# killerwhile/kafka-assignment-optimizer

Measured on AMD Instinct MI355X. Metric: candidate assignments/sec (+ time_to_optimal_s), 10k-partition reassign, higher is better.
Workload: dtype int32

## Files before the change

### kafka_assignment_optimizer_amd/csrc/kao_search.hip

```cpp
#include "kao_search_dev.h"

namespace kao {

template <bool kGlobalA, bool kPriced, int NW, bool kWide, bool kTeam, bool kCurG = false, int RFT = 0, bool kSmall = false>
__device__ __forceinline__ void search_body(unsigned char *smem, const SearchPools &pl, const SearchParams &prm) {
    static_assert(!kTeam || kGlobalA, "teams run topics that live in global memory");
    static_assert(!kCurG || !kGlobalA, "kCurG: the working assignment is in LDS");
    static_assert(RFT == 0 || (RFT == 3 && NW == 4 && !kGlobalA && !kTeam), "RFT = 3: LDS-resident topics of four words per partition");
    static_assert(!kSmall || (RFT == 3 && !kPriced && !kCurG), "kSmall: the unpriced RF-3 instantiation");
    constexpr int NS = RFT ? RFT : NW;
    const int lane = threadIdx.x & 63;
    const int wave = __builtin_amdgcn_readfirstlane(threadIdx.x >> 6);
    const int n_waves = kTeam ? __builtin_amdgcn_readfirstlane((int)(blockDim.x >> 6)) : 1;
    const int tid = kTeam ? (int)threadIdx.x : lane, nthr = kTeam ? (int)blockDim.x : 64;
    const int2 bm = pl.block_map[blockIdx.x];
    const TopicDev *TD = pl.topics + bm.x;

    TopicRegs T = topic_regs<RFT>(TD);
    {
        uint32_t v0 = T.c7_inc, v1 = T.c7_dec;
        asm volatile("" : "+v"(v0), "+v"(v1));
        T.c7_inc = (uint32_t)__builtin_amdgcn_readfirstlane((int)v0); T.c7_dec = (uint32_t)__builtin_amdgcn_readfirstlane((int)v1);
    }
    constexpr bool kBandTabs = kSmall;
// ... 157 lines not shown
    const int plog = TD->period_log2 + (rho & 3);
    const uint32_t pmask = (1u << plog) - 1u;
    const uint32_t lrange = (uint32_t)(prm.lam_max - prm.lam_min + 1);
    const uint32_t RF8 = (uint32_t)T.RF << 8, R8 = (uint32_t)T.R << 8, m8 = (uint32_t)T.m << 8;

    const int T_tour = min(64, max(4, (T.P * T.RF) >> 2));
    uint32_t tour_off = lane < T_tour ? 0u : kKeyNull;
    asm volatile("" : "+v"(tour_off));
    const int GA = min(16, max(1, (T.P * T.RF) >> 8));
    const int x_rounds_full = (T.P + 63) >> 6;
    const bool x_windowed = x_rounds_full > 8;

    int lam_lo = prm.lam_min, lam_hi = prm.lam_max;
    uint32_t n_iters = prm.iters, it_base = prm.launch * prm.iters;
    constexpr uint32_t kLpScanTwo = 1u << 29;
    uint32_t loop_pack = TD->P * TD->RF <= prm.scan2_max ? kLpScanTwo : 0u;
    if (kSmall) loop_pack |= ((uint32_t)prm.lam_min & 0xFFFu) | (((uint32_t)prm.lam_max & 0xFFFu) << 12) | (((uint32_t)plog & 31u) << 24);
    {
        uint32_t v0 = (uint32_t)lam_lo, v1 = (uint32_t)lam_hi, v2 = n_iters, v3 = it_base, v4 = loop_pack;
        asm volatile("" : "+v"(v2), "+v"(v3), "+v"(v4));
        if constexpr (!kSmall) {
            asm volatile("" : "+v"(v0), "+v"(v1));
            lam_lo = (int)__builtin_amdgcn_readfirstlane(v0); lam_hi = (int)__builtin_amdgcn_readfirstlane(v1);
        }
        n_iters = __builtin_amdgcn_readfirstlane(v2); it_base = __builtin_amdgcn_readfirstlane(v3);
        loop_pack = __builtin_amdgcn_readfirstlane(v4);
    }
    auto loop_flag = [&](uint32_t bit) { uint32_t lp = loop_pack; asm volatile("" : "+s"(lp)); return (lp & bit) != 0u; };
    constexpr bool kFuse = !kGlobalA && !kTeam && !kPriced;
    const bool fuse_ok = kFuse && T.Bx <= 16384;
    uint32_t jmp_a = 1u, jmp_c = 0u;
    if (fuse_ok)
        for (int n = (T.Bx + 63) >> 6; n > 0; --n) { jmp_a = (jmp_a * 0x6D2B79u) & 0xFFFFFFu; jmp_c = (jmp_c * 0x6D2B79u + 0x3C6EF3u) & 0xFFFFFFu; }
    best_obj = __builtin_amdgcn_readfirstlane(best_obj);
    for (uint32_t i = 0; i < n_iters; ++i) {
        const uint32_t it = it_base + i;
        const int type = (int)((0x1210u >> ((it & 7u) * 2u)) & 3u);
        int lam;
        if constexpr (kSmall) {
            uint32_t lp = loop_pack;
            asm volatile("" : "+s"(lp));
            const uint32_t plg = (lp >> 24) & 31u;
            const int lo_ = (int)(lp & 0xFFFu), hi_ = (int)((lp >> 12) & 0xFFFu);
            const uint32_t ph = it & ((1u << plg) - 1u);
            lam = best_obj < 0 ? hi_ : min(hi_, lo_ + (int)((2u * ph * (uint32_t)(hi_ - lo_ + 1)) >> plg));
        } else {
            const uint32_t ph = it & pmask;
            lam = best_obj < 0 ? lam_hi : min(lam_hi, lam_lo + (int)((2u * ph * lrange) >> plog));
        }
        const bool sampled = (type == 2) || (type == 0 && ((it >> 3) & 1u));

        auto finish = [&](auto ty, auto uni, uint32_t kmin, int win, int p, int k, int q, int j, uint32_t uw, uint32_t vw, int dV, int dObj) {
            constexpr int TY = decltype(ty)::value;
            auto of_win = [&](int v) { return decltype(uni)::value ? v : __builtin_amdgcn_readlane(v, win); };
            if (!kTeam) {
                if (kmin == kKeyNull) return;
                if ((int)(kmin >> 8) - kDBias > 0) return;
            }
            bool mine = true;
            int *rec = TR + ((i & 1u) * 16 + (uint32_t)wave) * kTeamRec;
            if (kTeam) {
                const bool ok = kmin != kKeyNull && (int)(kmin >> 8) - kDBias <= 0;
                if (lane == win) {
                    const uint32_t ro_ = uw >> 16, rn_ = vw >> 16;
                    const bool racks = ok && TY == 0 && ro_ != rn_;
                    rec[0] = ok ? 1 : 0; rec[1] = p; rec[2] = TY == 1 ? q : p;
                    rec[3] = (int)(uw & 0xFFFFu); rec[4] = (int)(vw & 0xFFFFu);
                    rec[5] = racks ? (int)ro_ : 0xFFFF; rec[6] = racks ? (int)rn_ : 0xFFFF;
                    rec[7] = dV; rec[8] = dObj;
                }
                __syncthreads();
                bool clash = false;
                if (lane < wave) {
                    const int *o = TR + ((i & 1u) * 16 + (uint32_t)lane) * kTeamRec;
                    if (o[0]) {
                        const int mp = rec[1], mq = rec[2], mb0 = rec[3], mb1 = rec[4], mr0 = rec[5], mr1 = rec[6];
                        clash = (o[1] == mp) | (o[1] == mq) | (o[2] == mp) | (o[2] == mq) | (o[3] == mb0) | (o[3] == mb1) | (o[4] == mb0) | (o[4] == mb1);
                        if (o[5] != 0xFFFF && mr0 != 0xFFFF) clash |= (o[5] == mr0) | (o[5] == mr1) | (o[6] == mr0) | (o[6] == mr1);
                    }
                }
                mine = ok && __ballot(clash) == 0ull;
            }

            if (lane == win && mine) {
                uint32_t *ap = reinterpret_cast<uint32_t *>(&L.A[p]);
                if (TY == 0) {
                    const uint32_t d = (k == 0) ? 0x10001u : 1u;
                    L.C[uw & 0xFFFFu] -= d;
                    L.C[vw & 0xFFFFu] += d;
                    if (!kTeam || (uw >> 16) != (vw >> 16)) {
                        L.K[uw >> 16] -= 1;
                        L.K[vw >> 16] += 1;
                    }
                    ap[k] = vw;
                } else if (TY == 1) {
                    uint32_t *bp = reinterpret_cast<uint32_t *>(&L.A[q]);
                    if ((k == 0) != (j == 0)) {
                        const uint32_t lose = (k == 0) ? uw : vw, gain = (k == 0) ? vw : uw;
                        L.C[lose & 0xFFFFu] -= 0x10000u;
                        L.C[gain & 0xFFFFu] += 0x10000u;
                    }
                    ap[k] = vw;
                    bp[j] = uw;
                } else {
                    L.C[uw & 0xFFFFu] -= 0x10000u;
                    L.C[vw & 0xFFFFu] += 0x10000u;
                    ap[0] = vw;
                    ap[k] = uw;
                }
            }
            if (mine) {
                int rows;
                if (TY == 0) rows = 1 | (of_win(k) == 0 ? 2 : 0);
                else if (TY == 1) rows = (of_win(k) == 0 ? 2 : 0) ^ (of_win(j) == 0 ? 2 : 0);
                else rows = 2;
                if (rows != 0) {
                    const uint32_t xo = (uint32_t)of_win((int)uw) & 0xFFFFu, xn = decltype(uni)::value ? (uint32_t)__builtin_amdgcn_readfirstlane((int)(vw & 0xFFFFu)) : (uint32_t)of_win((int)vw) & 0xFFFFu;
                    uint32_t xx = xo;
                    asm("v_writelane_b32 %0, %1, 1" : "+v"(xx) : "s"(xn));
                    int lane_w = lane;
                    asm volatile("" : "+v"(lane_w));
                    if (lane_w < 2) {
                        const uint32_t cx = L.C[xx];
                        uint32_t wx;
                        if (rows == 3) wx = band_row<kBandTabs>((int)(cx & 0xFFFFu), bq_r0, bq_r1) | (band_row<kBandTabs>((int)(cx >> 16), bq_l0, bq_l1) << 6);
                        else if (rows == 1) wx = (L.W[xx] & ~kWRowR) | band_row<kBandTabs>((int)(cx & 0xFFFFu), bq_r0, bq_r1);
                        else wx = (L.W[xx] & ~kWRowL) | (band_row<kBandTabs>((int)(cx >> 16), bq_l0, bq_l1) << 6);
                        L.W[xx] = (uint16_t)wx;
                    }
                }
            }
            if (kGlobalA) __builtin_amdgcn_fence(__ATOMIC_SEQ_CST, "workgroup");
            if (kTeam) {
                if (lane == 0) rec[9] = mine ? 1 : 0;
                __syncthreads();
                int dVs = 0, dOs = 0, na = 0;
                if (lane < n_waves) {
                    const int *o = TR + ((i & 1u) * 16 + (uint32_t)lane) * kTeamRec;
                    if (o[9]) { dVs = o[7]; dOs = o[8]; na = 1; }
                }
                V += wave_sum(dVs);
                obj += wave_sum(dOs);
                accepted += wave_sum(na);
            } else {
                V += of_win(dV);
                obj += of_win(dObj);
                accepted++;
            }
        };
        constexpr std::integral_constant<int, 0> kReplace{};
        constexpr std::integral_constant<int, 1> kExchange{};
        constexpr std::integral_constant<int, 2> kLeaderSwap{};

        if (sampled) {
            const int p = (int)rnd24_wide(rng, (uint32_t)T.P);
            const Part<NW> a = L.A[p];
            const Part<NW> c = CUR[p];
            uint32_t key = kKeyNull, vw = 0;
            int dV = 0, dObj = 0;
            if (type == 0) {
                const int k = (int)rnd24(rng, RF8);
                const uint32_t uw = sel_slot<NS>(a, k);
                const uint32_t ro = uw >> 16;
                const bool lead = k == 0;
                const uint32_t lw = lead ? 2u : 0u;
                const int wl = lead ? T.w00 : T.w01, wf = lead ? T.w10 : T.w11;
                const int g_old = role_w2<NS>(c, uw, wl, wf) + (hbw ? bw_of(BW[uw & 0xFFFFu], lead) : 0);
                const uint32_t wo = L.W[uw & 0xFFFFu];
                const int dV_old = wfld(wo, kWDecR) + wfldw(wo, kWDecL, lw);
                const int dV_rack_old = ddec(L.K[ro], T.rack_lo, T.rack_hi) + c7_delta(T.c7_dec, cnt4x2<NS>(a, ro));
                const int rsz_ro = RSZ[ro];
                int dP_old = 0, dP_rack_old = 0;
                if (kPriced) {
                    const uint32_t pro = PR[uw & 0xFFFFu];
                    dP_old = -(wflag(wo, kWPoutR) & price_rep(pro));
                    if (lead) dP_old -= wflag(wo, kWPoutL) & price_lead(pro);
                    dP_rack_old = p_out(L.K[ro], T.rack_lo, T.rack_hi, PG[ro]);
                }
                const int base_s = kSmall ? mad24s(S, g_old, kDBias) : 0;
#pragma unroll
                for (int g = 0; g < 4; ++g) {
                    uint32_t r, jj;
                    bool okg;
                    if (g < 2) {
                        r = rnd24(rng, R8);
                        jj = rnd24(rng, m8);
                        okg = (int)jj < RSZ[r];
                    } else {
                        r = ro;
                        jj = rnd24(rng, (uint32_t)rsz_ro << 8);
                        okg = true;
                    }
                    const uint32_t x = __umul24(r, (uint32_t)T.m) + jj;
                    const uint32_t xw = x | (r << 16);
                    okg = okg && !in4<NS>(a, xw);
                    const uint32_t wn = L.W[x];
                    int dVg = dV_old + wfld(wn, kWIncR) + wfldw(wn, kWIncL, lw);
                    if (g < 2) {
                        if (r != ro)
                            dVg += dV_rack_old + dinc(L.K[r], T.rack_lo, T.rack_hi) + c7_delta(T.c7_inc, cnt4x2<NS>(a, r));
                    }
                    const int dObjg = role_w2<NS>(c, xw, wl, wf) + (hbw ? bw_of(BW[x], lead) : 0) - (kSmall ? 0 : g_old);
                    uint32_t keyg;
                    if constexpr (kSmall) keyg = okg ? key_small(mad24s(-S, dObjg, mad24s(lam, dVg, base_s)), (uint32_t)lane) : kKeyNull;
                    else if (kPriced) {
                        const uint32_t prx = PR[x];
                        int dPg = dP_old + (wflag(wn, kWPinR) & price_rep(prx));
                        if (lead) dPg += wflag(wn, kWPinL) & price_lead(prx);
                        if (g < 2 && r != ro) dPg += dP_rack_old + p_in(L.K[r], T.rack_lo, T.rack_hi, PG[r]);
                        keyg = okg ? make_key_p(lam, S, dVg, dObjg, dPg, lane) : kKeyNull;
                    }
                    else keyg = okg ? make_key(lam, S, dVg, dObjg, lane) : kKeyNull;
                    if (keyg < key) { key = keyg; vw = xw; dV = dVg; dObj = dObjg; }
// ... 108 lines not shown
                    const int q_draw = (int)rnd24_wide(rng, (uint32_t)T.P);
                    q0 = x_windowed ? __builtin_amdgcn_readfirstlane(q_draw) : 0;
#pragma unroll
                    for (int r2 = 0; r2 < XB; ++r2) { int qq; bool okq; const int qc = x_partner(r2, qq, okq); xb[r2] = L.A[qc]; xcb[r2] = CUR[qc]; }
                }
#pragma unroll
                for (int g0 = 0; g0 < 16; g0 += TB) {
                    if (g0 > 0 && g0 >= GA) break;
                    Part<NW> tal[TB], tcl[TB];
                    int tp[TB];
#pragma unroll
                    for (int g = 0; g < TB; ++g) { tp[g] = (g0 + g) < GA ? part(g0 + g) : p0; tal[g] = L.A[tp[g]]; tcl[g] = CUR[tp[g]]; }
#pragma unroll
                    for (int g = 0; g < TB; ++g) {
                        uint32_t kg, ow;
                        int gg, d1 = 0, d2 = 0;
                        score_words(ty, kg, tal[g], tcl[g], kk[g0 + g], ow, gg, d1, d2);
                        if (g0 + g > 0) kg |= (g0 + g) < GA ? 0u : kKeyNull;
                        if (g0 + g == 0 || kg < keyA) { keyA = kg; pl_ = tp[g]; kl_ = kk[g0 + g]; oldw_l = ow; g_old_l = gg; dvo_l = d1; dvr_l = d2; a_l = tal[g]; c_l = tcl[g]; }
                    }
                }
            };
            if constexpr (kGlobalA) { if (type == 0) tournament_global(std::integral_constant<int, 0>{}); else tournament_global(std::integral_constant<int, 1>{}); }
            else if (type == 0) tournament(std::integral_constant<int, 0>{}); else tournament(std::integral_constant<int, 1>{});
            const int wA1 = (int)(wave_umin(keyA) & 63u);
            int wA2 = -1;
            if (type == 0 && loop_flag(kLpScanTwo)) {
                const uint32_t k2 = wave_umin(lane == wA1 ? kKeyNull : keyA);
                wA2 = k2 == kKeyNull ? -1 : (int)(k2 & 63u);
            }
            if (kFuse && type == 0 && wA2 >= 0 && fuse_ok) {
                int ps[2], ks[2], gs[2], dvos[2];
                uint32_t us[2];
                int v_rk[2];
#pragma unroll
                for (int s2 = 0; s2 < 2; ++s2) {
                    const int wA = s2 == 0 ? wA1 : wA2;
                    ps[s2] = __builtin_amdgcn_readlane(pl_, wA);
                    ks[s2] = __builtin_amdgcn_readlane(kl_, wA);
                    us[s2] = (uint32_t)__builtin_amdgcn_readlane((int)oldw_l, wA);
                    gs[s2] = __builtin_amdgcn_readlane(g_old_l, wA);
                    dvos[s2] = __builtin_amdgcn_readlane(dvo_l, wA);
                    v_rk[s2] = __builtin_amdgcn_readlane(dvr_l, wA);
                }
                const Part<NW> a1 = L.A[ps[0]], c1 = CUR[ps[0]], a2 = L.A[ps[1]], c2 = CUR[ps[1]];
                const uint32_t ro1 = us[0] >> 16, ro2 = us[1] >> 16;
                for (int r = lane; r < T.R; r += 64) {
                    const int dk = dinc(L.K[r], T.rack_lo, T.rack_hi);
                    const int v1 = ((uint32_t)r != ro1) ? v_rk[0] + dk + c7_delta(T.c7_inc, cnt4x2<NS>(a1, (uint32_t)r)) : 0;
                    const int v2 = ((uint32_t)r != ro2) ? v_rk[1] + dk + c7_delta(T.c7_inc, cnt4x2<NS>(a2, (uint32_t)r)) : 0;
                    L.RT[r] = kSmall ? (int)(((uint32_t)v2 & 0xFFFFu) | ((uint32_t)v1 << 16)) : (int)(((uint32_t)v1 & 0xFFFFu) | ((uint32_t)v2 << 16));
                }
                int lane_v = lane;
                asm volatile("" : "+v"(lane_v));
                const int li = lane_v & (NW - 1);
                const bool l2 = lane_v >= NW;
                const int p_l = l2 ? ps[1] : ps[0];
                const uint32_t ai = reinterpret_cast<const uint32_t *>(&L.A[p_l])[li], ci = reinterpret_cast<const uint32_t *>(&CUR[p_l])[li];
                const bool holds = (lane_v < 2 * NW) & (ai != kNoneW);
                uint32_t w_keep = 0;
                if (holds) w_keep = L.W[ai & 0xFFFFu];
                if (holds & !l2) L.W[ai & 0xFFFFu] = (uint16_t)(w_keep | kWNoCand);
                if (holds & l2) L.W[ai & 0xFFFFu] = (uint16_t)(L.W[ai & 0xFFFFu] | kWNoCand2);
                const bool hc = (lane_v < 2 * NW) & (ci != kNoneW);
                uint32_t w_ci = 0;
                if (hc) w_ci = L.W[ci & 0xFFFFu];
                const bool hm_l = hc & ((w_ci & (l2 ? kWNoCand2 : kWNoCand)) == 0u);
                const int mr_l = hm_l ? (int)((ci & 0xFFFFu) >> 6) : -1;
                int mr[2 * NW];
#pragma unroll
                for (int i2 = 0; i2 < 2 * NW; ++i2) mr[i2] = (i2 & (NW - 1)) < NS ? __builtin_amdgcn_readlane(mr_l, i2) : -1;
                const bool lead1 = ks[0] == 0, lead2 = ks[1] == 0;
                const uint32_t lw1 = lead1 ? 2u : 0u, lw2 = lead2 ? 2u : 0u;
                const int wl1 = lead1 ? T.w00 : T.w01, wf1 = lead1 ? T.w10 : T.w11, wl2 = lead2 ? T.w00 : T.w01, wf2 = lead2 ? T.w10 : T.w11;
                const int K01 = __mul24(S, gs[0]) + kDBias + __mul24(lam, dvos[0]);
                const int K02 = __mul24(S, gs[1]) + kDBias + __mul24(lam, dvos[1]);
                const uint32_t leadp = (lead2 ? 1u : 0u) | (lead1 ? 0x10000u : 0u);
                const uint32_t K0p = ((uint32_t)K02 & 0xFFFFu) | ((uint32_t)K01 << 16);
                const int wl1h = (int)((uint32_t)(S * wl1) << 16), wf1h = (int)((uint32_t)(S * wf1) << 16);
                const int wl2s = (int)((uint32_t)(S * wl2) & 0xFFFFu), wf2s = (int)((uint32_t)(S * wf2) & 0xFFFFu);
                uint32_t jc = jmp_c;
                asm volatile("" : "+v"(jc));
                uint32_t best1 = kKeyNull, best2 = kKeyNull;
                auto scan_round2 = [&](auto with_w, int base, int rd, uint32_t &key1, uint32_t &key2) {
                    const uint32_t st1 = lcg24(rng);
                    uint32_t st2;
                    asm("v_mad_u32_u24 %0, %1, %2, %3" : "=v"(st2) : "v"(st1), "s"(jmp_a), "v"(jc));
                    const int w = (int)reinterpret_cast<const short *>(L.W)[base + lane];
                    const int rt = L.RT[XR[base + lane]];
                    const int inc = wfld(w, kWIncR);
                    if constexpr (kSmall) {
                        uint32_t d = pk_mad_ss(pk_add(pk_mad_lo((uint32_t)wfld(w, kWIncL), leadp, (uint32_t)inc), (uint32_t)rt), (uint32_t)lam, K0p);
                        if (decltype(with_w)::value) {
                            const uint32_t x = (uint32_t)(base + lane);
                            const uint32_t xw = x | ((uint32_t)XR[x] << 16);
                            auto mask_of = [](bool b) { uint32_t m = b ? ~0u : 0u; asm("" : "+v"(m)); return m; };
                            const bool l1 = c1.w[0] == xw, l2 = c2.w[0] == xw;
                            bool f1 = false, f2 = false;
#pragma unroll
                            for (int i2 = 1; i2 < NS; ++i2) { f1 |= c1.w[i2] == xw; f2 |= c2.w[i2] == xw; }
                            auto and_or = [](uint32_t m, uint32_t w, uint32_t acc) { uint32_t r; asm("v_and_or_b32 %0, %1, %2, %3" : "=v"(r) : "v"(m), "s"(w), "v"(acc)); return r; };
                            uint32_t ws = mask_of(l1) & (uint32_t)wl1h;
                            ws = and_or(mask_of(f1), (uint32_t)wf1h, ws);
                            ws = and_or(mask_of(l2), (uint32_t)wl2s, ws);
                            ws = and_or(mask_of(f2), (uint32_t)wf2s, ws);
                            d = pk_sub(d, ws);
                        }
                        key1 = ((d | (uint32_t)w) & 0xFFFF0000u) | (st1 & 0xFF00u) | (uint32_t)rd;
                        key2 = ((d | (uint32_t)wflag(w, 14)) << 16) | (st2 & 0xFF00u) | (uint32_t)rd;
                        return;
                    }
                    int d1 = __mul24(lam, inc + wfldw(w, kWIncL, lw1) + wfldw(rt, 0, 16u)) + K01;
                    int d2 = __mul24(lam, inc + wfldw(w, kWIncL, lw2) + (rt >> 16)) + K02;
                    if (decltype(with_w)::value) {
                        const uint32_t x = (uint32_t)(base + lane);
                        const uint32_t xw = x | ((uint32_t)XR[x] << 16);
                        d1 -= __mul24(S, role_w2<NS>(c1, xw, wl1, wf1));
                        d2 -= __mul24(S, role_w2<NS>(c2, xw, wl2, wf2));
                    }
                    d1 = min(max(d1, 0), 2 * kDBias - 2);
                    d2 = min(max(d2, 0), 2 * kDBias - 2) | wflag(w, 14);
                    key1 = ((uint32_t)d1 << 16) | (st1 & 0xFF00u) | (uint32_t)rd | ((uint32_t)w & 0xFFFF0000u);
                    key2 = ((uint32_t)d2 << 16) | (st2 & 0xFF00u) | (uint32_t)rd;
                };
                const int n_rd = (T.Bx + 63) >> 6;
                int rd = 0, base = 0;
                while (rd < n_rd) {
                    int nxt = n_rd;
#pragma unroll
                    for (int i2 = 0; i2 < 2 * NW; ++i2)
                        if (mr[i2] >= rd) nxt = min(nxt, mr[i2]);
                    uint32_t k1a, k2a, k1b, k2b;
                    for (; rd + 1 < nxt; rd += 2, base += 128) {
                        scan_round2(std::false_type{}, base, rd, k1a, k2a);
                        scan_round2(std::false_type{}, base + 64, rd + 1, k1b, k2b);
                        best1 = min(best1, min(k1a, k1b));
                        best2 = min(best2, min(k2a, k2b));
                    }
                    if (rd < nxt) { scan_round2(std::false_type{}, base, rd, k1a, k2a); best1 = min(best1, k1a); best2 = min(best2, k2a); ++rd; base += 64; }
                    if (rd < n_rd) { scan_round2(std::true_type{}, base, rd, k1a, k2a); best1 = min(best1, k1a); best2 = min(best2, k2a); ++rd; base += 64; }
                }
                asm("v_mad_u32_u24 %0, %0, %1, %2" : "+v"(rng) : "s"(jmp_a), "v"(jc));
                if (holds) L.W[ai & 0xFFFFu] = (uint16_t)w_keep;
                const uint32_t kw = wave_umin(min(((best1 >> 1) & ~127u) | (uint32_t)lane, ((best2 >> 1) & ~127u) | 64u | (uint32_t)lane));
                const bool two = (kw & 64u) != 0u;
                const uint32_t kmin = kw >> 7;
                const int win = (int)(kw & 63u);
                const int p = two ? ps[1] : ps[0], k = two ? ks[1] : ks[0];
                const uint32_t uw = two ? us[1] : us[0];
                if ((int)(kmin >> 8) - kDBias <= 0) {
                    const bool lead = k == 0;
                    const uint32_t bw_ = (uint32_t)__builtin_amdgcn_readlane((int)(two ? best2 : best1), win);
                    const uint32_t xs = ((bw_ & 255u) << 6) + (uint32_t)win;
                    const uint32_t rs = XR[xs];
                    const uint32_t ws = L.W[xs];
                    const int rts = L.RT[rs];
                    const uint32_t vw = xs | (rs << 16);
                    const int dV = wfld(ws, kWIncR) + wfldw(ws, kWIncL, lead ? 2u : 0u) + (two ? dvos[1] : dvos[0]) + ((two != kSmall) ? (rts >> 16) : wfldw(rts, 0, 16u));
                    int mx1 = -1, mx2 = -1;
#pragma unroll
                    for (int i2 = 0; i2 < NW; ++i2) { mx1 = max(mx1, mr[i2]); mx2 = max(mx2, mr[NW + i2]); }
                    const bool has_missing = (two ? mx2 : mx1) >= 0;
                    const int dObj = -(two ? gs[1] : gs[0]) + (has_missing ? (two ? role_w2<NS>(c2, vw, wl2, wf2) : role_w2<NS>(c1, vw, wl1, wf1)) : 0);
                    finish(kReplace, std::true_type{}, kmin, win, p, k, 0, 0, uw, vw, dV, dObj);
                }
            } else {
            auto slot_of = [&](int wA, int &p, int &k, uint32_t &uw, int &g_old, int &dV_old, int &dV_rack_old, Part<NW> &a, Part<NW> &c) {
                p = __builtin_amdgcn_readlane(pl_, wA);
                k = __builtin_amdgcn_readlane(kl_, wA);
                uw = (uint32_t)__builtin_amdgcn_readlane((int)oldw_l, wA);
                g_old = __builtin_amdgcn_readlane(g_old_l, wA);
                dV_old = __builtin_amdgcn_readlane(dvo_l, wA);
                dV_rack_old = __builtin_amdgcn_readlane(dvr_l, wA);
                if constexpr (kGlobalA) {
#pragma unroll
                    for (int i2 = 0; i2 < NW; ++i2) { a.w[i2] = (uint32_t)__builtin_amdgcn_readlane((int)a_l.w[i2], wA); c.w[i2] = (uint32_t)__builtin_amdgcn_readlane((int)c_l.w[i2], wA); }
                } else {
                    a = L.A[p];
                    c = CUR[p];
                }
            };
            if (type == 0) {
            uint32_t b_kmin = kKeyNull, b_uw = 0, b_vw = 0;
            int b_win = 0, b_p = 0, b_k = 0, b_dV = 0, b_dObj = 0;
#pragma nounroll
            for (int si = 0; si < (wA2 >= 0 ? 2 : 1); ++si) {
                int p, k, g_old, dV_old, dV_rack_old;
                uint32_t uw;
                Part<NW> a, c;
                slot_of(si == 0 ? wA1 : wA2, p, k, uw, g_old, dV_old, dV_rack_old, a, c);
                const bool lead = k == 0;
                const uint32_t ro = uw >> 16;
                uint32_t vw = 0;
                int dV = 0, dObj = 0;
                {
                    const int dP_rack_old = kPriced ? p_out(L.K[ro], T.rack_lo, T.rack_hi, PG[ro]) : 0;
                    for (int r = lane; r < T.R; r += 64) {
                        int v = ((uint32_t)r != ro) ? dV_rack_old + dinc(L.K[r], T.rack_lo, T.rack_hi) + c7_delta(T.c7_inc, cnt4x2<NS>(a, (uint32_t)r)) : 0;
                        if (kPriced)
                            v = (v & 0xFF) | ((((uint32_t)r != ro) ? dP_rack_old + p_in(L.K[r], T.rack_lo, T.rack_hi, PG[r]) : 0) * 256);
                        L.RT[r] = v;
                    }
                }
                const int wl = lead ? T.w00 : T.w01, wf = lead ? T.w10 : T.w11;
                const int li = lane & (NW - 1);
                const uint32_t ai = sel_slot<NS>(a, li), ci = sel_slot<NS>(c, li);
                const bool holds = (lane < NS) & (ai != kNoneW);
                uint32_t w_keep = 0;
                if (!kTeam && holds) {
                    w_keep = L.W[ai & 0xFFFFu];
                    L.W[ai & 0xFFFFu] = (uint16_t)(w_keep | kWNoCand);
                }
                int ar[NS];
                {
                    const int ar_l = (kTeam && holds) ? (int)((ai & 0xFFFFu) >> 6) : -1;
#pragma unroll
                    for (int i2 = 0; i2 < NS; ++i2) ar[i2] = __builtin_amdgcn_readlane(ar_l, i2);
                }
                const bool hm_l = (lane < NS) & (ci != kNoneW) & !in4<NS>(a, ci);
                const int mr_l = hm_l ? (int)((ci & 0xFFFFu) >> 6) : -1;
                int mr[NS];
#pragma unroll
                for (int i2 = 0; i2 < NS; ++i2) mr[i2] = __builtin_amdgcn_readlane(mr_l, i2);
                bool has_missing = false;
#pragma unroll
                for (int i2 = 0; i2 < NS; ++i2) has_missing |= mr[i2] >= 0;
                int K0 = __mul24(S, g_old) + kDBias + __mul24(lam, dV_old);
                if (kPriced) {
                    const uint32_t pro = PR[uw & 0xFFFFu];
                    const uint32_t wo = L.W[uw & 0xFFFFu];
                    K0 -= wflag(wo, kWPoutR) & price_rep(pro);
                    if (lead) K0 -= wflag(wo, kWPoutL) & price_lead(pro);
                }
                const uint32_t lw = lead ? 2u : 0u, lf = lead ? 1u : 0u;
                uint32_t bestA = kKeyNull;
                int chunkA = 0;
                auto scan_round = [&](auto with_w, int base, int rd) -> uint32_t {
                    const uint32_t st = lcg24(rng);
                    const int w = (int)(short)L.W[base + lane];
                    const int rt = L.RT[XR[base + lane]];
                    int dsc;
                    if (kPriced) {
                        const uint32_t prx = PR[base + lane];
                        const int dVx = wfld(w, kWIncR) + wfldw(w, kWIncL, lw) + (int)(signed char)(rt & 0xFF);
                        dsc = __mul24(lam, dVx) + K0 + (rt >> 8) + (wflag(w, kWPinR) & price_rep(prx)) + (wflagw(w, kWPinL, lf) & price_lead(prx));
                        if (hbw) dsc -= __mul24(S, bw_of(BW[base + lane], lead));
                    } else {
                        const int dVx = wfld(w, kWIncR) + wfldw(w, kWIncL, lw) + rt;
                        dsc = __mul24(lam, dVx) + K0;
                    }
                    uint32_t member = 0;
                    if (decltype(with_w)::value) {
                        const uint32_t x = (uint32_t)(base + lane);
                        const uint32_t xw = x | ((uint32_t)XR[x] << 16);
                        dsc -= __mul24(S, role_w2<NS>(c, xw, wl, wf));
                        if (kTeam && in4<NS>(a, xw)) member = 0xFFFF0000u;
                    }
                    dsc = min(max(dsc, 0), 2 * kDBias - 2);
                    return ((uint32_t)dsc << 16) | (st & 0xFF00u) | (uint32_t)rd | ((uint32_t)w & 0xFFFF0000u) | member;
                };
                auto is_weighted = [&](int rdg) {
                    bool wgt = false;
#pragma unroll
                    for (int i2 = 0; i2 < NS; ++i2) wgt |= (mr[i2] == rdg) | (kTeam && ar[i2] == rdg);
                    return wgt;
                };
                for (int cb = 0; cb < T.Bx; cb += 16384) {
                    uint32_t bestc = kKeyNull;
                    const int cend = min(T.Bx, cb + 16384);
                    int rd = 0, base = cb;
                    if (kWide) {
                        for (; base + 64 < cend; base += 128, rd += 2) {
                            const int rdg = (cb >> 6) + rd;
                            if (is_weighted(rdg) || is_weighted(rdg + 1)) {
                                bestc = min(bestc, is_weighted(rdg) ? scan_round(std::true_type{}, base, rd) : scan_round(std::false_type{}, base, rd));
                                bestc = min(bestc, is_weighted(rdg + 1) ? scan_round(std::true_type{}, base + 64, rd + 1) : scan_round(std::false_type{}, base + 64, rd + 1));
                            } else {
                                const uint32_t k0 = scan_round(std::false_type{}, base, rd);
                                const uint32_t k1 = scan_round(std::false_type{}, base + 64, rd + 1);
                                bestc = min(bestc, min(k0, k1));
                            }
                        }
                    }
                    if (kWide || kTeam) {
                        for (; base < cend; base += 64, ++rd)
                            bestc = min(bestc, is_weighted((cb >> 6) + rd) ? scan_round(std::true_type{}, base, rd) : scan_round(std::false_type{}, base, rd));
                    } else {
                        const int n_rd = (cend - cb + 63) >> 6, rd0 = cb >> 6;
                        while (rd < n_rd) {
                            int nxt = n_rd;
#pragma unroll
                            for (int i2 = 0; i2 < NS; ++i2) {
                                const int m = mr[i2] - rd0;
                                if (m >= rd) nxt = min(nxt, m);
                            }
                            for (; rd + 1 < nxt; rd += 2, base += 128) {
                                const uint32_t k0 = scan_round(std::false_type{}, base, rd);
                                const uint32_t k1 = scan_round(std::false_type{}, base + 64, rd + 1);
                                bestc = min(bestc, min(k0, k1));
                            }
                            if (rd < nxt) { bestc = min(bestc, scan_round(std::false_type{}, base, rd)); ++rd; base += 64; }
                            if (rd < n_rd) { bestc = min(bestc, scan_round(std::true_type{}, base, rd)); ++rd; base += 64; }
                        }
                    }
                    if ((bestc >> 8) < (bestA >> 8)) { bestA = bestc; chunkA = cb; }
                }
                if (!kTeam && holds) L.W[ai & 0xFFFFu] = (uint16_t)w_keep;
                const uint32_t key = bestA >> 8;
                const uint32_t kmin = wave_umin(key);
                const unsigned long long bal = __ballot(key == kmin);
                const int win = __ffsll((long long)bal) - 1;
                if ((int)(kmin >> 8) - kDBias <= 0) {
                    const uint32_t bw_ = (uint32_t)__builtin_amdgcn_readlane((int)bestA, win);
                    const uint32_t xs = (uint32_t)__builtin_amdgcn_readlane(chunkA, win) + ((bw_ & 255u) << 6) + (uint32_t)win;
                    const uint32_t rs = XR[xs];
                    const uint32_t ws = L.W[xs];
                    const int rts = L.RT[rs];
                    vw = xs | (rs << 16);
                    dV = wfld(ws, kWIncR) + wfldw(ws, kWIncL, lw) + dV_old + (kPriced ? (int)(signed char)(rts & 0xFF) : rts);
                    dObj = -g_old + (has_missing ? role_w2<NS>(c, vw, wl, wf) : 0) + (hbw ? bw_of(BW[xs], lead) : 0);
                }
                if (si == 0 || kmin < b_kmin) { b_kmin = kmin; b_win = win; b_p = p; b_k = k; b_uw = uw; b_vw = vw; b_dV = dV; b_dObj = dObj; }
            }
            finish(kReplace, std::true_type{}, b_kmin, b_win, b_p, b_k, 0, 0, b_uw, b_vw, b_dV, b_dObj);
            } else {
                int p, k, g_old, dV_old, dV_rack_old;
                uint32_t uw;
                Part<NW> a, c;
                slot_of(wA1, p, k, uw, g_old, dV_old, dV_rack_old, a, c);
                const bool lead = k == 0;
                const uint32_t ro = uw >> 16;
                uint32_t key = kKeyNull, vw = 0;
                int dV = 0, dObj = 0, q = 0, j = 0;
                const int nrp = lead ? 0 : 1;
                const int cnt_a_ru2 = cnt4x2<NS>(a, ro);
                const uint32_t wu = L.W[uw & 0xFFFFu];
                const int pl_u = kPriced ? price_lead(PR[uw & 0xFFFFu]) : 0;
                const int bwl_u = hbw ? (int)(BW[uw & 0xFFFFu] >> 16) : 0;
                if (!kGlobalA) {
                    const int q_draw = (int)rnd24_wide(rng, (uint32_t)T.P);
                    q0 = x_windowed ? __builtin_amdgcn_readfirstlane(q_draw) : 0;
                }
                const int x_rounds = x_windowed ? 8 : x_rounds_full;
                auto x_round = [&](int rd, const Part<NW> &b, const Part<NW> &cb) {
                    const uint32_t tie0 = lcg24(rng) >> 8;
                    int qq; bool okq;
                    x_partner(rd, qq, okq);
                    okq = okq & (qq != p);
                    const bool u_in_b = in4<NS>(b, uw);
                    const int u_in_q_lead = role_w2<NS>(cb, uw, T.w00, T.w10), u_in_q_fol = role_w2<NS>(cb, uw, T.w01, T.w11);
                    const int dv_ro = c7_delta(T.c7_dec, cnt_a_ru2) + c7_delta(T.c7_inc, cnt4x2<NS>(b, ro));
                    int cnt_b_rv[3] = {0, 0, 0};
                    if constexpr (RFT == 3) {
                        const int e01 = (int)((b.w[0] >> 16) == (b.w[1] >> 16)), e02 = (int)((b.w[0] >> 16) == (b.w[2] >> 16)), e12 = (int)((b.w[1] >> 16) == (b.w[2] >> 16));
                        cnt_b_rv[0] = (1 + e01 + e02) << 1; cnt_b_rv[1] = (1 + e01 + e12) << 1; cnt_b_rv[2] = (1 + e02 + e12) << 1;
                    }
#pragma unroll
                    for (int jj = 0; jj < NS; ++jj) {
                        if (!RFT && jj >= T.RF) break;
                        const uint32_t v = b.w[jj];
                        const bool ok = okq & (v != uw) & !in4<NS>(a, v) & !u_in_b;
                        const int nrq = jj != 0;
                        int dObjx = role_w<NS>(T, c, v, nrp) + (jj == 0 ? u_in_q_lead : u_in_q_fol) - g_old - role_w<NS>(T, cb, v, nrq);
                        int dVx = 0, dPx = 0;
                        if (lead != (jj == 0)) {
                            const uint32_t wv = L.W[v & 0xFFFFu];
                            dVx += lead ? (wfld(wu, kWDecL) + wfld(wv, kWIncL)) : (wfld(wv, kWDecL) + wfld(wu, kWIncL));
                            if (kPriced) {
                                if (hbw) { const int dbl = (int)(BW[v & 0xFFFFu] >> 16) - bwl_u; dObjx += lead ? dbl : -dbl; }
                                const int plv = price_lead(PR[v & 0xFFFFu]);
                                dPx = lead ? ((wflag(wv, kWPinL) & plv) - (wflag(wu, kWPoutL) & pl_u))
                                           : ((wflag(wu, kWPinL) & pl_u) - (wflag(wv, kWPoutL) & plv));
                            }
                        }
                        const uint32_t rv = v >> 16;
                        if (rv != ro)
                            dVx += dv_ro + c7_delta(T.c7_inc, cnt4x2<NS>(a, rv)) + c7_delta(T.c7_dec, RFT == 3 ? cnt_b_rv[jj < 3 ? jj : 0] : cnt4x2<NS>(b, rv));
                        uint32_t keyx;
                        if constexpr (kSmall) keyx = ok ? key_small(mad24s(lam, dVx, mad24s(-S, dObjx, kDBias)), (tie0 + (uint32_t)jj * 0x55u) & 0xFFu) : kKeyNull;
                        else if (kPriced) keyx = ok ? make_key_tie_p(lam, S, dVx, dObjx, dPx, tie0 + (uint32_t)jj * 0x55u) : kKeyNull;
                        else keyx = ok ? make_key_tie(lam, S, dVx, dObjx, tie0 + (uint32_t)jj * 0x55u) : kKeyNull;
                        if (keyx < key) { key = keyx; vw = v; q = qq; j = jj; dV = dVx; dObj = dObjx; }
                    }
// ... 303 lines not shown
```

### kafka_assignment_optimizer_amd/csrc/kao_search_dev.h

```cpp
#pragma once
#include <hip/hip_runtime.h>

#include <type_traits>

#include "kao_device.h"
#include "kao_internal.h"

namespace kao {

__device__ __forceinline__ uint32_t fmix32(uint32_t h) {
    h ^= h >> 16; h *= 0x85EBCA6Bu; h ^= h >> 13; h *= 0xC2B2AE35u; h ^= h >> 16;
    return h;
}
__device__ __forceinline__ uint32_t xs32(uint32_t &s) {
    s ^= s << 13; s ^= s >> 17; s ^= s << 5;
    return s;
}
__device__ __forceinline__ uint32_t mulhi(uint32_t a, uint32_t b) { return __umulhi(a, b); }
__device__ __forceinline__ int band(int c, int lo, int hi) { return max(c - hi, 0) + max(lo - c, 0); }
__device__ __forceinline__ int dinc(int c, int lo, int hi) { return (int)(c >= hi) - (int)(c < lo); }
__device__ __forceinline__ int ddec(int c, int lo, int hi) { return (int)(c <= lo) - (int)(c > hi); }

template <int NW> struct alignas(16) Part { uint32_t w[NW]; };
__device__ __forceinline__ uint32_t sel4(const Part<4> &a, int k) {
// ... 185 lines not shown
    const int pin = (b >= 0 || a < 0) ? 1 : 0, pout = (b > 0 || a <= 0) ? 1 : 0;
    return (unsigned long long)((di & 3) | ((dd & 3) << 2) | (pin << 4) | (pout << 5));
}
constexpr unsigned long long band_table() {
    unsigned long long t = 0;
    for (int a = -1; a <= 1; ++a) for (int b = -1; b <= 1; ++b) t |= band_entry_of(a, b) << (6 * (3 * (a + 1) + (b + 1)));
    return t;
}
constexpr unsigned long long kBandTab = band_table();
__device__ __forceinline__ int clamp_pm1(int x) {
    int r;
    asm("v_med3_i32 %0, %1, -1, 1" : "=v"(r) : "v"(x));
    return r;
}
__device__ __forceinline__ uint32_t band_entry(int c, int lo, int hi) {
    const int a = clamp_pm1(c - lo), b = clamp_pm1(c - hi);
    int t;
    asm("v_mad_i32_i24 %0, %1, 3, %2" : "=v"(t) : "v"(a), "v"(b));
    return (uint32_t)(kBandTab >> (uint32_t)(__mul24(t, 6) + 24)) & 63u;
}
constexpr int kBandTabLast = 4;
constexpr bool band_tab_fits(int lo, int hi) { return lo >= 0 && lo <= hi && hi <= 0xFFFF && hi - lo + 2 <= kBandTabLast; }
constexpr uint32_t band_tab(int lo, int hi) {
    uint32_t t = 0;
    for (int i = 0; i <= kBandTabLast; ++i) {
        const int c = lo - 1 + (i < hi - lo + 2 ? i : hi - lo + 2);
        const int a = c < lo ? -1 : (c > lo ? 1 : 0), b = c < hi ? -1 : (c > hi ? 1 : 0);
        t |= (uint32_t)band_entry_of(a, b) << (6 * i);
    }
    return t;
}
constexpr int band_tab_bias(int lo) { return 6 - 6 * lo; }
constexpr uint32_t band_lookup_plain(int c, int bias, uint32_t tab) {
    const int x = 6 * c + bias;
    return (tab >> (x < 0 ? 0 : (x > 6 * kBandTabLast ? 6 * kBandTabLast : x))) & 63u;
}
__device__ __forceinline__ uint32_t band_lookup(int c, int bias, uint32_t tab) {
    int x;
    asm("v_mad_i32_i24 %0, %1, 6, %2\n\tv_med3_i32 %0, %0, 0, 24" : "=&v"(x) : "v"(c), "v"(bias));
    static_assert(6 * kBandTabLast == 24, "the clamp's inline constant");
    return __builtin_amdgcn_ubfe(tab, (uint32_t)x, 6u);
}
template <bool kTab> __device__ __forceinline__ uint32_t band_row(int c, int r0, int r1) {
    if constexpr (kTab) return band_lookup(c, r0, (uint32_t)r1);
    else return band_entry(c, r0, r1);
}
__device__ __forceinline__ uint32_t band_fields(const TopicRegs &T, uint32_t c) {
    return band_entry((int)(c & 0xFFFFu), T.rep_lo, T.rep_hi) | (band_entry((int)(c >> 16), T.lead_lo, T.lead_hi) << 6);
}
constexpr uint32_t kWRowR = 0x003Fu, kWRowL = 0x0FC0u;
constexpr uint32_t kWNoCand = 0x8000u;
constexpr uint32_t kWNoCand2 = 0x4000u;
template <int NW> __device__ __forceinline__ void rebuild_band_state(const TopicRegs &T, const WaveLds<NW> &L, const uint8_t *XR, uint32_t inv, int lane, int stride = 64) {
    for (int x = lane; x < ((T.Bx + 63) & ~63); x += stride) L.W[x] = (uint16_t)(XR[x] == inv ? (kWNoCand | kWNoCand2) : band_fields(T, L.C[x]));
}

struct FillTabs {
    uint16_t *W;
    const uint8_t *XR;
    const int *K;
    int *RT;
    const uint32_t *PR;
    const int *PG;
    const uint32_t *BW;
};
constexpr uint32_t kFillTieStep = 0x165667B1u;
template <int NS, int NW> __device__ __forceinline__ void fill_mark(uint16_t *W, const Part<NW> &a, int lane) {
    const uint32_t ai = sel_slot<NS>(a, lane & (NW - 1));
    if ((lane < NS) & (ai != kNoneW)) W[ai & 0xFFFFu] |= (uint16_t)kWNoCand;
}
template <int NS, int NW> __device__ __forceinline__ void fill_unmark(uint16_t *W, const Part<NW> &a, int lane) {
    const uint32_t ai = sel_slot<NS>(a, lane & (NW - 1));
    if ((lane < NS) & (ai != kNoneW)) W[ai & 0xFFFFu] &= (uint16_t)~kWNoCand;
}
template <int NS, bool kPriced, int NW> __device__ __forceinline__ void fill_rack_table(const TopicRegs &T, const FillTabs &F, const Part<NW> &a, int lane) {
    for (int r = lane; r < T.R; r += 64) {
        const int kr = F.K[r];
        int v = dinc(kr, T.rack_lo, T.rack_hi) + c7_delta(T.c7_inc, cnt4x2<NS>(a, (uint32_t)r));
        if (kPriced) v = (v & 0xFF) | (p_in(kr, T.rack_lo, T.rack_hi, F.PG[r]) * 256);
        F.RT[r] = v;
    }
}
template <int NS, bool kPriced, bool kClamp, bool kWithW, int NW>
__device__ __forceinline__ uint32_t fill_round(const TopicRegs &T, const FillTabs &F, const Part<NW> &c, int x, int rd, uint32_t h, int lam, int S, bool lead) {
    const int w = (int)reinterpret_cast<const short *>(F.W)[x];
    const uint32_t r = F.XR[x];
    const int rt = F.RT[r];
    const uint32_t lw = lead ? 2u : 0u, lf = lead ? 1u : 0u;
    int cost;
    if (kPriced) {
        const uint32_t prx = F.PR[x];
        const int dVx = wfld(w, kWIncR) + wfldw(w, kWIncL, lw) + (int)(signed char)(rt & 0xFF);
        cost = __mul24(lam, dVx) + kDBias + (rt >> 8) + (wflag(w, kWPinR) & price_rep(prx)) + (wflagw(w, kWPinL, lf) & price_lead(prx));
        if (F.BW) cost -= __mul24(S, bw_of(F.BW[x], lead));
    } else {
        cost = mad24s(lam, wfld(w, kWIncR) + wfldw(w, kWIncL, lw) + rt, kDBias);
    }
    if (kWithW) cost -= __mul24(S, role_w2<NS>(c, (uint32_t)x | (r << 16), lead ? T.w00 : T.w01, lead ? T.w10 : T.w11));
    if (kClamp) cost = min(max(cost, 0), 2 * kDBias - 2);
    h ^= h >> 16; h *= 0x85EBCA6Bu; h ^= h >> 13; h *= 0xC2B2AE35u;
    return ((uint32_t)cost << 16) | ((h >> 16) & 0xFF00u) | (uint32_t)rd | ((uint32_t)w & 0xFFFF0000u);
}
template <int NS, bool kPriced, bool kClamp, bool kWeights, int NW>
__device__ __forceinline__ uint32_t fill_hole(const TopicRegs &T, const FillTabs &F, const Part<NW> &a, const Part<NW> &c, bool lead, uint32_t hmix, int lam, int S, int lane) {
    fill_rack_table<NS, kPriced>(T, F, a, lane);
    int mr[NS] = {};
    if constexpr (kWeights) {
        const uint32_t ci = sel_slot<NS>(c, lane & (NW - 1));
        const int mr_l = ((lane < NS) & (ci != kNoneW) & !in4<NS>(a, ci)) ? (int)((ci & 0xFFFFu) >> 6) : -1;
#pragma unroll
        for (int i = 0; i < NS; ++i) mr[i] = __builtin_amdgcn_readlane(mr_l, i);
    }
    uint32_t h = hmix + (uint32_t)lane * kFillTieStep;
    uint32_t best = kKeyNull;
    int chunk = 0;
    for (int cb = 0; cb < T.Bx; cb += 16384) {
        uint32_t bestc = kKeyNull;
        const int n_rd = (min(T.Bx, cb + 16384) - cb + 63) >> 6;
        int rd = 0, x = cb + lane;
        if constexpr (!kWeights) {
            for (; rd + 1 < n_rd; rd += 2, x += 128, h += 128u * kFillTieStep) {
                const uint32_t k0 = fill_round<NS, kPriced, kClamp, false>(T, F, c, x, rd, h, lam, S, lead);
                const uint32_t k1 = fill_round<NS, kPriced, kClamp, false>(T, F, c, x + 64, rd + 1, h + 64u * kFillTieStep, lam, S, lead);
                bestc = min(bestc, min(k0, k1));
            }
            if (rd < n_rd) { bestc = min(bestc, fill_round<NS, kPriced, kClamp, false>(T, F, c, x, rd, h, lam, S, lead)); h += 64u * kFillTieStep; }
        } else {
            for (; rd < n_rd; ++rd, x += 64, h += 64u * kFillTieStep) {
                bool wgt = false;
#pragma unroll
                for (int i = 0; i < NS; ++i) wgt |= mr[i] == (cb >> 6) + rd;
                bestc = min(bestc, wgt ? fill_round<NS, kPriced, kClamp, true>(T, F, c, x, rd, h, lam, S, lead) : fill_round<NS, kPriced, kClamp, false>(T, F, c, x, rd, h, lam, S, lead));
            }
        }
        if ((bestc >> 8) < (best >> 8)) { best = bestc; chunk = cb; }
    }
    const uint32_t m = wave_umin(((best >> 1) & ~127u) | (uint32_t)lane);
    if ((m >> 15) == 0xFFFFu) return kNoneW;
    const int win = (int)(m & 63u);
    const uint32_t bw = (uint32_t)__builtin_amdgcn_readlane((int)best, win);
    const uint32_t xs = (uint32_t)__builtin_amdgcn_readlane(chunk, win) + ((bw & 255u) << 6) + (uint32_t)win;
    return xs | ((uint32_t)F.XR[xs] << 16);
}

template <int NW> __device__ __forceinline__ void recount(const TopicRegs &T, const WaveLds<NW> &L, int lane, int stride, int krt) {
    for (int x = lane; x < ((T.Bx + 63) & ~63); x += stride) L.C[x] = 0;
    for (int r = lane; r < krt; r += stride) L.K[r] = 0;
    if (stride > 64) __syncthreads();
    for (int p = lane; p < T.P; p += stride) {
        const Part<NW> a = L.A[p];
#pragma unroll
        for (int k = 0; k < NW; ++k)
            if (a.w[k] != kNoneW) { atomicAdd(&L.C[a.w[k] & 0xFFFFu], k == 0 ? 0x10001u : 1u); atomicAdd(&L.K[a.w[k] >> 16], 1); }
    }
}

template <int NW, bool kTeam = false> __device__ __forceinline__ void full_cost(const TopicRegs &T, const WaveLds<NW> &L, const Part<NW> *CUR, const int *RSZ,
                                                            int lane, int stride, int &V, int &obj, const uint32_t *BW = nullptr,
                                                            int *TS = nullptr, int wave = 0, int n_waves = 1) {
    int v = 0, o = 0;
    for (int p = lane; p < T.P; p += stride) {
        const Part<NW> a = L.A[p];
        const Part<NW> c = CUR[p];
#pragma unroll
        for (int k = 0; k < NW; ++k)
            if (a.w[k] != kNoneW) o += role_w(T, c, a.w[k], k == 0 ? 0 : 1);
        v += part_rack_viol(T, a);
    }
    for (int x = lane; x < T.Bx; x += stride) {
        const int r = (int)mulhi((uint32_t)x, T.magic);
        if (x - r * T.m < RSZ[r]) {
            const uint32_t c = L.C[x];
            v += band((int)(c & 0xFFFFu), T.rep_lo, T.rep_hi) + band((int)(c >> 16), T.lead_lo, T.lead_hi);
            if (BW) { const uint32_t bw = BW[x]; o += (int)(c & 0xFFFFu) * (int)(bw & 0xFFFFu) + (int)(c >> 16) * (int)(bw >> 16); }
        }
    }
    for (int r = lane; r < T.R; r += stride) v += band(L.K[r], T.rack_lo, T.rack_hi);
    V = wave_sum(v);
    obj = wave_sum(o);
    if (kTeam) {
        __syncthreads();
        if ((lane & 63) == 0) { TS[2 * wave] = V; TS[2 * wave + 1] = obj; }
        __syncthreads();
        int tv = 0, to = 0;
        if ((lane & 63) < n_waves) { tv = TS[2 * (lane & 63)]; to = TS[2 * (lane & 63) + 1]; }
        V = wave_sum(tv);
        obj = wave_sum(to);
    }
}

template <int NW> __device__ __forceinline__ void snapshot(const TopicRegs &T, const WaveLds<NW> &L, const uint16_t *ext, uint16_t *best, int lane, int stride = 64) {
    int p0 = 0;
    do {
        const int p = p0 + lane;
        if (p < T.P) {
            const Part<NW> a = L.A[p];
            uint16_t *o = best + p * T.RF;
#pragma unroll
            for (int k = 0; k < NW; ++k)
                if (k < T.RF) o[k] = ext[a.w[k] & 0xFFFFu];
        }
        p0 += stride;
    } while (p0 < T.P);
}

}
// ... 1 lines not shown
```

Baseline: 906.2 billion.

## Fuse single-wave accept update into one LDS trip and batch scan loads

For the unpriced RF-3 single-wave instantiation, the accept step now writes the assignment and updates broker counts, rack counts and band rows in one pass. Up to four lanes each own one counter instead of a single lane doing serial read-modify-writes. Separately, the paired scan and fill loops now issue both rounds' LDS loads (weights, rack index, rack table) before computing either round, so the two dependent gathers can overlap. The fused path drops the `mine` guard and the team-specific rack-count condition, so it relies on the single-wave case always accepting.

After: 918.8 billion, median of 6. +1.4%, better.

```diff
diff --git a/kafka_assignment_optimizer_amd/csrc/kao_search.hip b/kafka_assignment_optimizer_amd/csrc/kao_search.hip
--- a/kafka_assignment_optimizer_amd/csrc/kao_search.hip
+++ b/kafka_assignment_optimizer_amd/csrc/kao_search.hip
@@ -263,6 +263,52 @@
                 mine = ok && __ballot(clash) == 0ull;
             }
 
+            constexpr bool kOneTrip = !kTeam && kSmall;
+            if constexpr (kOneTrip) {
+                if (lane == win) {
+                    uint32_t *ap = reinterpret_cast<uint32_t *>(&L.A[p]);
+                    if (TY == 0) ap[k] = vw;
+                    else if (TY == 1) { ap[k] = vw; reinterpret_cast<uint32_t *>(&L.A[q])[j] = uw; }
+                    else { ap[0] = vw; ap[k] = uw; }
+                }
+                const int kw = of_win(k);
+                int rows;
+                if (TY == 0) rows = 1 | (kw == 0 ? 2 : 0);
+                else if (TY == 1) rows = (kw == 0 ? 2 : 0) ^ (of_win(j) == 0 ? 2 : 0);
+                else rows = 2;
+                if (rows != 0) {
+                    const uint32_t uws = (uint32_t)of_win((int)uw);
+                    const uint32_t vws = decltype(uni)::value ? (uint32_t)__builtin_amdgcn_readfirstlane((int)vw) : (uint32_t)of_win((int)vw);
+                    const uint32_t xo = uws & 0xFFFFu, xn = vws & 0xFFFFu;
+                    uint32_t xx = xo;
+                    asm("v_writelane_b32 %0, %1, 1" : "+v"(xx) : "s"(xn));
+                    uint32_t xi = xx;
+                    const uint32_t d0 = TY == 0 ? (kw == 0 ? 0x10001u : 1u) : (TY == 1 ? (kw == 0 ? 0x10000u : 0u - 0x10000u) : 0x10000u);
+                    int n_own = 2;
+                    if (TY == 0) {
+                        const uint32_t ro_ = uws >> 16, rn_ = vws >> 16;
+                        asm("v_writelane_b32 %0, %1, 2\n\tv_writelane_b32 %0, %2, 3" : "+v"(xi) : "s"(ro_), "s"(rn_));
+                        n_own = ro_ != rn_ ? 4 : 2;
+                    }
+                    int lane_w = lane;
+                    asm volatile("" : "+v"(lane_w));
+                    if (lane_w < n_own) {
+                        uint32_t *cp = (lane_w < 2 ? L.C : reinterpret_cast<uint32_t *>(L.K)) + xi;
+                        const uint32_t c_old = *cp;
+                        const uint32_t w_old = L.W[xx];
+                        const uint32_t dl = lane_w < 2 ? d0 : 1u;
+                        const uint32_t cx = (lane_w & 1) ? c_old + dl : c_old - dl;
+                        *cp = cx;
+                        if (lane_w < 2) {
+                            uint32_t wx;
+                            if (rows == 3) wx = band_row<kBandTabs>((int)(cx & 0xFFFFu), bq_r0, bq_r1) | (band_row<kBandTabs>((int)(cx >> 16), bq_l0, bq_l1) << 6);
+                            else if (rows == 1) wx = (w_old & ~kWRowR) | band_row<kBandTabs>((int)(cx & 0xFFFFu), bq_r0, bq_r1);
+                            else wx = (w_old & ~kWRowL) | (band_row<kBandTabs>((int)(cx >> 16), bq_l0, bq_l1) << 6);
+                            L.W[xx] = (uint16_t)wx;
+                        }
+                    }
+                }
+            } else {
             if (lane == win && mine) {
                 uint32_t *ap = reinterpret_cast<uint32_t *>(&L.A[p]);
                 if (TY == 0) {
@@ -310,6 +356,7 @@
                         L.W[xx] = (uint16_t)wx;
                     }
                 }
+            }
             }
             if (kGlobalA) __builtin_amdgcn_fence(__ATOMIC_SEQ_CST, "workgroup");
             if (kTeam) {
@@ -584,12 +631,11 @@
                 uint32_t jc = jmp_c;
                 asm volatile("" : "+v"(jc));
                 uint32_t best1 = kKeyNull, best2 = kKeyNull;
-                auto scan_round2 = [&](auto with_w, int base, int rd, uint32_t &key1, uint32_t &key2) {
+                const short *Ws = reinterpret_cast<const short *>(L.W);
+                auto scan_round2 = [&](auto with_w, int base, int rd, int w, int rt, uint32_t &key1, uint32_t &key2) {
                     const uint32_t st1 = lcg24(rng);
                     uint32_t st2;
                     asm("v_mad_u32_u24 %0, %1, %2, %3" : "=v"(st2) : "v"(st1), "s"(jmp_a), "v"(jc));
-                    const int w = (int)reinterpret_cast<const short *>(L.W)[base + lane];
-                    const int rt = L.RT[XR[base + lane]];
                     const int inc = wfld(w, kWIncR);
                     if constexpr (kSmall) {
                         uint32_t d = pk_mad_ss(pk_add(pk_mad_lo((uint32_t)wfld(w, kWIncL), leadp, (uint32_t)inc), (uint32_t)rt), (uint32_t)lam, K0p);
@@ -634,13 +680,16 @@
                         if (mr[i2] >= rd) nxt = min(nxt, mr[i2]);
                     uint32_t k1a, k2a, k1b, k2b;
                     for (; rd + 1 < nxt; rd += 2, base += 128) {
-                        scan_round2(std::false_type{}, base, rd, k1a, k2a);
-                        scan_round2(std::false_type{}, base + 64, rd + 1, k1b, k2b);
+                        const int wa = Ws[base + lane], wb = Ws[base + 64 + lane];
+                        const uint32_t ra = XR[base + lane], rb = XR[base + 64 + lane];
+                        const int rta = L.RT[ra], rtb = L.RT[rb];
+                        scan_round2(std::false_type{}, base, rd, wa, rta, k1a, k2a);
+                        scan_round2(std::false_type{}, base + 64, rd + 1, wb, rtb, k1b, k2b);
                         best1 = min(best1, min(k1a, k1b));
                         best2 = min(best2, min(k2a, k2b));
                     }
-                    if (rd < nxt) { scan_round2(std::false_type{}, base, rd, k1a, k2a); best1 = min(best1, k1a); best2 = min(best2, k2a); ++rd; base += 64; }
-                    if (rd < n_rd) { scan_round2(std::true_type{}, base, rd, k1a, k2a); best1 = min(best1, k1a); best2 = min(best2, k2a); ++rd; base += 64; }
+                    if (rd < nxt) { const int wa = Ws[base + lane]; scan_round2(std::false_type{}, base, rd, wa, L.RT[XR[base + lane]], k1a, k2a); best1 = min(best1, k1a); best2 = min(best2, k2a); ++rd; base += 64; }
+                    if (rd < n_rd) { const int wa = Ws[base + lane]; scan_round2(std::true_type{}, base, rd, wa, L.RT[XR[base + lane]], k1a, k2a); best1 = min(best1, k1a); best2 = min(best2, k2a); ++rd; base += 64; }
                 }
                 asm("v_mad_u32_u24 %0, %0, %1, %2" : "+v"(rng) : "s"(jmp_a), "v"(jc));
                 if (holds) L.W[ai & 0xFFFFu] = (uint16_t)w_keep;
@@ -737,10 +786,9 @@
                 const uint32_t lw = lead ? 2u : 0u, lf = lead ? 1u : 0u;
                 uint32_t bestA = kKeyNull;
                 int chunkA = 0;
-                auto scan_round = [&](auto with_w, int base, int rd) -> uint32_t {
+                const short *Ws = reinterpret_cast<const short *>(L.W);
+                auto scan_round_on = [&](auto with_w, int base, int rd, int w, int rt) -> uint32_t {
                     const uint32_t st = lcg24(rng);
-                    const int w = (int)(short)L.W[base + lane];
-                    const int rt = L.RT[XR[base + lane]];
                     int dsc;
                     if (kPriced) {
                         const uint32_t prx = PR[base + lane];
@@ -760,6 +808,18 @@
                     }
                     dsc = min(max(dsc, 0), 2 * kDBias - 2);
                     return ((uint32_t)dsc << 16) | (st & 0xFF00u) | (uint32_t)rd | ((uint32_t)w & 0xFFFF0000u) | member;
+                };
+                auto scan_round = [&](auto with_w, int base, int rd) -> uint32_t {
+                    const int w = Ws[base + lane];
+                    return scan_round_on(with_w, base, rd, w, L.RT[XR[base + lane]]);
+                };
+                auto scan_pair = [&](int base, int rd) -> uint32_t {
+                    const int wa = Ws[base + lane], wb = Ws[base + 64 + lane];
+                    const uint32_t ra = XR[base + lane], rb = XR[base + 64 + lane];
+                    const int rta = L.RT[ra], rtb = L.RT[rb];
+                    const uint32_t k0 = scan_round_on(std::false_type{}, base, rd, wa, rta);
+                    const uint32_t k1 = scan_round_on(std::false_type{}, base + 64, rd + 1, wb, rtb);
+                    return min(k0, k1);
                 };
                 auto is_weighted = [&](int rdg) {
                     bool wgt = false;
@@ -777,11 +837,7 @@
                             if (is_weighted(rdg) || is_weighted(rdg + 1)) {
                                 bestc = min(bestc, is_weighted(rdg) ? scan_round(std::true_type{}, base, rd) : scan_round(std::false_type{}, base, rd));
                                 bestc = min(bestc, is_weighted(rdg + 1) ? scan_round(std::true_type{}, base + 64, rd + 1) : scan_round(std::false_type{}, base + 64, rd + 1));
-                            } else {
-                                const uint32_t k0 = scan_round(std::false_type{}, base, rd);
-                                const uint32_t k1 = scan_round(std::false_type{}, base + 64, rd + 1);
-                                bestc = min(bestc, min(k0, k1));
-                            }
+                            } else bestc = min(bestc, scan_pair(base, rd));
                         }
                     }
                     if (kWide || kTeam) {
@@ -796,11 +852,7 @@
                                 const int m = mr[i2] - rd0;
                                 if (m >= rd) nxt = min(nxt, m);
                             }
-                            for (; rd + 1 < nxt; rd += 2, base += 128) {
-                                const uint32_t k0 = scan_round(std::false_type{}, base, rd);
-                                const uint32_t k1 = scan_round(std::false_type{}, base + 64, rd + 1);
-                                bestc = min(bestc, min(k0, k1));
-                            }
+                            for (; rd + 1 < nxt; rd += 2, base += 128) bestc = min(bestc, scan_pair(base, rd));
                             if (rd < nxt) { bestc = min(bestc, scan_round(std::false_type{}, base, rd)); ++rd; base += 64; }
                             if (rd < n_rd) { bestc = min(bestc, scan_round(std::true_type{}, base, rd)); ++rd; base += 64; }
                         }
diff --git a/kafka_assignment_optimizer_amd/csrc/kao_search_dev.h b/kafka_assignment_optimizer_amd/csrc/kao_search_dev.h
--- a/kafka_assignment_optimizer_amd/csrc/kao_search_dev.h
+++ b/kafka_assignment_optimizer_amd/csrc/kao_search_dev.h
@@ -291,10 +291,7 @@
     }
 }
 template <int NS, bool kPriced, bool kClamp, bool kWithW, int NW>
-__device__ __forceinline__ uint32_t fill_round(const TopicRegs &T, const FillTabs &F, const Part<NW> &c, int x, int rd, uint32_t h, int lam, int S, bool lead) {
-    const int w = (int)reinterpret_cast<const short *>(F.W)[x];
-    const uint32_t r = F.XR[x];
-    const int rt = F.RT[r];
+__device__ __forceinline__ uint32_t fill_round_on(const TopicRegs &T, const FillTabs &F, const Part<NW> &c, int x, int rd, uint32_t h, int lam, int S, bool lead, int w, uint32_t r, int rt) {
     const uint32_t lw = lead ? 2u : 0u, lf = lead ? 1u : 0u;
     int cost;
     if (kPriced) {
@@ -310,6 +307,12 @@
     h ^= h >> 16; h *= 0x85EBCA6Bu; h ^= h >> 13; h *= 0xC2B2AE35u;
     return ((uint32_t)cost << 16) | ((h >> 16) & 0xFF00u) | (uint32_t)rd | ((uint32_t)w & 0xFFFF0000u);
 }
+template <int NS, bool kPriced, bool kClamp, bool kWithW, int NW>
+__device__ __forceinline__ uint32_t fill_round(const TopicRegs &T, const FillTabs &F, const Part<NW> &c, int x, int rd, uint32_t h, int lam, int S, bool lead) {
+    const int w = (int)reinterpret_cast<const short *>(F.W)[x];
+    const uint32_t r = F.XR[x];
+    return fill_round_on<NS, kPriced, kClamp, kWithW>(T, F, c, x, rd, h, lam, S, lead, w, r, F.RT[r]);
+}
 template <int NS, bool kPriced, bool kClamp, bool kWeights, int NW>
 __device__ __forceinline__ uint32_t fill_hole(const TopicRegs &T, const FillTabs &F, const Part<NW> &a, const Part<NW> &c, bool lead, uint32_t hmix, int lam, int S, int lane) {
     fill_rack_table<NS, kPriced>(T, F, a, lane);
@@ -329,8 +332,11 @@
         int rd = 0, x = cb + lane;
         if constexpr (!kWeights) {
             for (; rd + 1 < n_rd; rd += 2, x += 128, h += 128u * kFillTieStep) {
-                const uint32_t k0 = fill_round<NS, kPriced, kClamp, false>(T, F, c, x, rd, h, lam, S, lead);
-                const uint32_t k1 = fill_round<NS, kPriced, kClamp, false>(T, F, c, x + 64, rd + 1, h + 64u * kFillTieStep, lam, S, lead);
+                const int wa = (int)reinterpret_cast<const short *>(F.W)[x], wb = (int)reinterpret_cast<const short *>(F.W)[x + 64];
+                const uint32_t ra = F.XR[x], rb = F.XR[x + 64];
+                const int rta = F.RT[ra], rtb = F.RT[rb];
+                const uint32_t k0 = fill_round_on<NS, kPriced, kClamp, false>(T, F, c, x, rd, h, lam, S, lead, wa, ra, rta);
+                const uint32_t k1 = fill_round_on<NS, kPriced, kClamp, false>(T, F, c, x + 64, rd + 1, h + 64u * kFillTieStep, lam, S, lead, wb, rb, rtb);
                 bestc = min(bestc, min(k0, k1));
             }
             if (rd < n_rd) { bestc = min(bestc, fill_round<NS, kPriced, kClamp, false>(T, F, c, x, rd, h, lam, S, lead)); h += 64u * kFillTieStep; }
```
